# AER-RC/monoRTM

Measured on AMD Instinct MI355X. Metric: (wavenumber x layer x line) optical-depth evals/sec, higher is better.
Workload: dtype f64; 1 GPU; c4: configs[3] whole: 1024 synthetic sonde profiles x 64 layers x 50 channels x 500 lines, f64, profile-sharded over 1 GPU(s): 1024 profiles on this rank; layers=64, wavenumbers=50, lines=500, nmol=7, launch=3 stream launches, parallelism=profile-sharded x1

## Files before the change

monortm_amd/csrc/api.hip:

```cpp
#include <algorithm>
#include <atomic>
#include <chrono>
#include <cmath>
#include <cstdlib>
#include <cstdio>
#include <cstring>
#include <dlfcn.h>
#include <functional>
#include <string>
#include <vector>

#include "device_common.hpp"
#include "line_table.hpp"
#include "modm_plan.hpp"
#include "lineshape.hpp"
#include "tables/monortm_tables.h"

namespace {
using namespace monortm_dev;

thread_local std::string g_init_error;

struct Ctx {
    int device = 0;
    int cus = 256;
    size_t phys_cap = 2ull << 30, far_cap = 1ull << 30;
    std::vector<Ctx *> shards;
    struct Opt : ModmPlanOpt {
        int ms_ablate = 0;
        int ms_prepare = MS_PREPARE_FUSED;
        double jac_dt = MONORTM_JAC_DT, jac_dlnw = MONORTM_JAC_DLNW;
    } opt;
    void *comm = nullptr;
    int comm_rank = 0, comm_world = 1;
    bool has_lines = false;
    int real_kind = 8;
    std::string err;
    monortm::LineTable host;
    DevLines lines{};
    DevTables tables{};
    std::vector<void *> owned;
    int *errflag = nullptr;
    void *partial = nullptr;
    monortm_dev::MwCache mw_cache;
    void *phys = nullptr;
    size_t phys_bytes = 0;
    void *far = nullptr;
    size_t far_bytes = 0;
    double lines_per_cm = 0.;
    bool no_physics_pass = false;
    hipStream_t far_stream = nullptr;
    hipEvent_t far_ev[2] = {nullptr, nullptr};
    double lc_frac = 0.;
    const int *ms_slot_base = nullptr;
    int ms_slot_host[MXMOL + 1] = {0};
    void *ms_scratch = nullptr;
    unsigned short *ms_reach = nullptr;
    size_t ms_scratch_bytes = 0;
    double *osum = nullptr;
    size_t osum_elems = 0;
    DevXsec xs{};
    std::vector<void *> xs_buf;
    struct Stage {
        void *p = nullptr;
        size_t bytes = 0;
    };
    Stage stage[12];
    void *jac_ws = nullptr;
    size_t jac_ws_bytes = 0;
    struct Obs {
        int handle = 0;
        int npath = 0, nwn = 0, nview = 0, nchan = 0;
        void *dev = nullptr;
// ... 74 lines not shown
    bool isint = false, isdbl = false;
    if (!autov) {
        char *end = nullptr;
        iv = strtol(v.c_str(), &end, 10);
        isint = end && end != v.c_str() && *end == '\0';
        end = nullptr;
        dv = strtod(v.c_str(), &end);
        isdbl = end && end != v.c_str() && *end == '\0';
    }
    if (n == "nslice" && (autov || (isint && iv >= 1 && iv <= 16))) c->opt.nslice = autov ? 0 : (int)iv;
    else if (n == "fair" && (autov || (isint && (iv == 0 || iv == 1)))) c->opt.fair = autov ? -1 : (int)iv;
    else if (n == "tile_waves" && (autov || (isint && (iv == 1 || iv == 2 || iv == 4)))) c->opt.tile_waves = autov ? 0 : (int)iv;
    else if (n == "far_levels" && (autov || (isint && iv >= 0 && iv <= FAR_MAXLEV))) c->opt.far_levels = autov ? -1 : (int)iv;
    else if (n == "lines_kernel" && (autov || v == "wn" || v == "ms")) c->opt.lines_ms = autov ? -1 : (v == "ms" ? 1 : 0);
    else if (n == "ms_prepare" && (autov || v == "fused" || v == "passes")) c->opt.ms_prepare = v == "passes" ? MS_PREPARE_PASSES : MS_PREPARE_FUSED;
#ifdef MONORTM_EXPERIMENT
    else if (n == "ms_ablate" && isint && iv >= 0 && iv <= 9) c->opt.ms_ablate = (int)iv;
#endif
    else if (n == "finish" && (autov || v == "generic")) c->opt.finish_generic = autov ? 0 : 1;
    else if (n == "ms_items" && (autov || (isint && (iv == 64 || iv == 128 || iv == 192 || iv == 256)))) c->opt.ms_items = autov ? 0 : (int)iv;
    else if ((n == "jac_dt" || n == "jac_dlnw") && (autov || (isdbl && std::isfinite(dv) && dv > 0. && (n == "jac_dt" || dv < 1.)))) {
        if (n == "jac_dt") c->opt.jac_dt = autov ? MONORTM_JAC_DT : dv;
        else c->opt.jac_dlnw = autov ? MONORTM_JAC_DLNW : dv;
    }
    else { c->err = "unknown option or value: " + n + " = " + v; return MONORTM_EARG; }
    return MONORTM_OK;
}

template <class T>
int upload(Ctx *c, const T *src, size_t n, const T **dst) {
// ... 691 lines not shown
        }
        if (hipGetLastError() != hipSuccess || hipDeviceSynchronize() != hipSuccess) { c->err = "log-ratio tables could not be formed"; return failed(MONORTM_EHIP); }
    }
    void *ef = nullptr;
    if (hipMalloc(&ef, sizeof(int)) != hipSuccess || hipMemset(ef, 0, sizeof(int)) != hipSuccess) { c->err = "hipMalloc(errflag) failed"; return failed(MONORTM_EHIP); }
    c->owned.push_back(ef);
    c->errflag = static_cast<int *>(ef);
    if (hipDeviceSynchronize() != hipSuccess) { c->err = "device set-up failed"; return failed(MONORTM_EHIP); }
    if (hipStreamCreateWithFlags(&c->hs, hipStreamNonBlocking) != hipSuccess ||
        hipHostMalloc(reinterpret_cast<void **>(&c->errflag_host), sizeof(int), hipHostMallocDefault) != hipSuccess) {
        c->err = "stream / pinned flag of the host-buffer entry points could not be created";
        return failed(MONORTM_EHIP);
    }
    if (const char *e = getenv("MONORTM_HOST_TIMING")) c->host_timing = e[0] == '1';
    if (getenv("MONORTM_FINISH_GENERIC")) c->opt.finish_generic = 1;
    for (const char *k : {"lines_kernel", "nslice", "fair", "tile_waves", "far_levels", "ms_items", "ms_prepare",
#ifdef MONORTM_EXPERIMENT
                          "ms_ablate",
#endif
                         }) {
        std::string env = "MONORTM_" + std::string(k);
        for (char &ch : env) ch = (char)toupper((unsigned char)ch);
        if (const char *e = getenv(env.c_str()))
            if (set_option(c, k, e)) { c->err = env + ": " + c->err; return failed(MONORTM_EARG); }
    }
    if (c->host_timing && !g_timing_ctx) {
        g_timing_ctx = c;
        static bool registered = false;
        if (!registered) { atexit([] { if (g_timing_ctx) print_host_timing(g_timing_ctx); }); registered = true; }
    }
    *out = c;
// ... 9 lines not shown
        return;
    }
    print_host_timing(c);
    if (g_timing_ctx == c) g_timing_ctx = nullptr;
    DeviceGuard guard;
    hipSetDevice(c->device);
    for (auto &e : c->events) { hipEventDestroy(e.a); hipEventDestroy(e.b); }
    for (auto &e : c->event_pool) hipEventDestroy(e);
    comm_release(c);
    if (c->hs) hipStreamDestroy(c->hs);
    if (c->errflag_host) hipHostFree(c->errflag_host);
    for (void *p : c->owned) hipFree(p);
    if (c->partial) hipFree(c->partial);
    if (c->osum) hipFree(c->osum);
    if (c->ms_scratch) hipFree(c->ms_scratch);
    for (void *p : c->xs_buf) hipFree(p);
    if (c->phys) hipFree(c->phys);
    if (c->far) hipFree(c->far);
    if (c->far_stream) hipStreamDestroy(c->far_stream);
    for (hipEvent_t e : c->far_ev)
        if (e) hipEventDestroy(e);
    c->mw_cache.release();
    if (c->jac_ws) hipFree(c->jac_ws);
    for (auto &ob : c->obs)
        if (ob.dev) hipFree(ob.dev);
    for (int i = 0; i < 12; i++)
        if (c->stage[i].p) {
            if (i % 2 == 0) hipHostFree(c->stage[i].p);
            else hipFree(c->stage[i].p);
        }
// ... 386 lines not shown
    if (pl.use_ms) {
        HIPCHK(c, grow(&c->ms_scratch, &c->ms_scratch_bytes, lines_ms_scratch(ms, (long long)ms.npg * nlay_max)));
        const size_t nl4 = (std::max<size_t>(c->host.size(), 1) + 3) / 4 * 4;
        if (!c->ms_reach) {
            void *p = nullptr;
            HIPCHK(c, hipMalloc(&p, 6 * nl4));
            c->owned.push_back(p);
            c->ms_reach = static_cast<unsigned short *>(p);
        }
        ms.reach = c->ms_reach;
        ms.near0 = reinterpret_cast<float *>(c->ms_reach + nl4);
        ms.scratch = c->ms_scratch;
        ms.slot_base = c->ms_slot_base;
        ms.ablate = c->opt.ms_ablate;
        ms.prepare = c->opt.ms_prepare;
    }
    const dim3 grid(pl.grid[0], pl.grid[1], pl.grid[2]);
    if (pl.use_ms && pl.ms_nprof < nprof) {
        ModmArgs am = a, aw = a;
        am.nprof = pl.ms_nprof;
        const size_t st = (size_t)pl.ms_nprof * nlay_max;
        auto shift = [](const void *p, size_t elems) { return p ? static_cast<const void *>(static_cast<const double *>(p) + elems) : nullptr; };
        aw.nprof = nprof - pl.ms_nprof;
        aw.P = shift(a.P, st); aw.T = shift(a.T, st); aw.CLW = shift(a.CLW, st); aw.WBRODL = shift(a.WBRODL, st);
        aw.WKL = shift(a.WKL, st * nmol);
        aw.nlay = a.nlay + pl.ms_nprof;
        aw.O = const_cast<void *>(shift(a.O, st * nwn)); aw.O_CLW = const_cast<void *>(shift(a.O_CLW, st * nwn));
        aw.O_BY_MOL = const_cast<void *>(shift(a.O_BY_MOL, st * nmol * nwn));
        aw.OC = const_cast<void *>(shift(a.OC, st * MONORTM_NCONT * nwn));
        aw.osum = a.osum ? a.osum + st * nwn : nullptr;
// ... 888 lines not shown
```

monortm_amd/csrc/device_common.hpp:

```cpp
#pragma once
#include <hip/hip_runtime.h>

#if (defined(FAR_ABL_HOT) || defined(FAR_ABL_STEPS) || defined(FAR_ABL_TRANS) || defined(MONORTM_ABLATE_LOOP) || defined(MONORTM_ABLATE_EVAL) || \
     defined(MONORTM_ABLATE_VOIGT) || defined(MONORTM_ABLATE_ZSEARCH) || defined(MONORTM_ABLATE_EXP4) || defined(MONORTM_ABLATE_COUPLE) ||     \
     defined(MONORTM_NO_CLAMP_GUARD) || defined(MONORTM_NO_UNIFIED) || defined(MONORTM_NO_VSCAN) ||              \
     defined(MONORTM_NO_HALF) || defined(MONORTM_NO_FULL) || defined(MONORTM_NO_CHUNKFAR) || defined(MONORTM_NO_SGL_TSKIP) || defined(LINES_TIMING) || \
     defined(LINES_CLASS_STATS) || defined(MW_TIMING)) &&                                                                                          \
    !defined(MONORTM_EXPERIMENT)
#error "a timing-experiment / A-B switch of monortm_amd is defined: such builds are measurements, not the product - add -DMONORTM_EXPERIMENT=1"
#endif

#include <cstdint>

#include "../../include/monortm_hip.h"

namespace monortm_dev {

#define K_PI 3.1415926535898
#define K_PLANCK 6.62606876E-27
#define K_BOLTZ 1.3806503E-16
#define K_CLIGHT 2.99792458E+10
#define K_AVOGAD 6.02214199E+23
#define K_RADCN1 1.191042722E-12
#define K_RADCN2 1.4387752
// ... 263 lines not shown
constexpr int MS_HOTA_BYTES = 32;
struct MsArgs {
    int G, LPS, CL, nsteps;
    int spp;
    int sa_stride;
    int npg;
    int nslot;
    int inv_cl;
    int inv_lps;
    const int *slot_base;
    void *scratch;
    unsigned short *reach;
    float *near0;
    int ablate;
    int prepare;
};
#define MS_PREPARE_FUSED 0
#define MS_PREPARE_PASSES 1
size_t lines_ms_scratch(const MsArgs &ms, long long nwg);
void launch_lines_ms(const ModmArgs &a, const DevLines &L, const DevTables &tb, const MsArgs &ms, bool ibrd, hipStream_t s);

void launch_physics(const ModmArgs &a, const DevLines &L, const DevTables &tb, int nlines, bool ibrd, hipStream_t s);
void launch_far_plan(const ModmArgs &a, const DevLines &L, const DevTables &tb, hipStream_t s);
void launch_far(const ModmArgs &a, const DevLines &L, const DevTables &tb, double rho_tile, double lines_per_cm, long long *launches,
                hipStream_t s);
void launch_lines(const ModmArgs &a, const DevLines &L, const DevTables &tb, int nw, int wpl, bool ibrd, dim3 grid, size_t dyn_lds,
                  hipStream_t s);
hipError_t launch_finish(const ModmArgs &a, const DevTables &tb, double V1ABS, double V2ABS, int NPTABS, int csize, bool high,
                         bool par, int threads, size_t lds, int lds_sets, hipStream_t s);
void launch_reduce_slices(const ModmArgs &a, hipStream_t s);
void launch_logratio(const double *t296, const double *tlow, double *out, int n, hipStream_t s);
struct MwCache {
    struct Entry {
// ... 28 lines not shown
```

monortm_amd/csrc/lines_ms_kernel.hip:

```cpp
#define MONORTM_EXP_SGPR_CONSTANTS 1
#include "lines_device.hpp"
#include "lines_ms_asm.hpp"
#include "modm_plan.hpp"
#include "ms_reach.hpp"

namespace {
using namespace monortm_dev;

constexpr int WPS = MS_WPS;
#if defined(MONORTM_ABLATE_EXP4) || defined(MONORTM_ABLATE_ZSEARCH) || defined(MONORTM_ABLATE_VOIGT) || defined(MONORTM_NO_CLAMP_GUARD)
constexpr bool MS_HAS_TRIP = false;
#else
constexpr bool MS_HAS_TRIP = true;
#endif
static_assert(MS_REACH_SLOTS == MS_WPS, "ms_reach.hpp forms one bit per wavenumber of a lane");

__device__ __forceinline__ void ms_sync() {
    __builtin_amdgcn_fence(__ATOMIC_RELEASE, "wavefront");
    __builtin_amdgcn_wave_barrier();
    __builtin_amdgcn_fence(__ATOMIC_ACQUIRE, "wavefront");
}
__device__ __forceinline__ void ms_sync_global() {
    __builtin_amdgcn_fence(__ATOMIC_RELEASE, "workgroup");
    __builtin_amdgcn_s_waitcnt(0);
// ... 7 lines not shown
    const ColdLine *gC;
    int item0;
};
struct MsSpec { unsigned long long w[MS_MAXSTEPS]; };
__device__ __forceinline__ bool ms_own(const MsSpec &sp, int item) {
    unsigned long long x = sp.w[0];
#pragma unroll
    for (int t = 1; t < MS_MAXSTEPS; t++) x = ((item >> 6) == t) ? sp.w[t] : x;
    return (x >> (item & 63)) & 1ull;
}
__device__ __forceinline__ HotB ms_hotb(const MsState &st, const MsSpec &sp, int j, const HotA &h) {
    if (ms_own(sp, st.item0 + j)) return st.gB[j];
    return HotB{h.pa, -1., 0., 1.};
}

template <int KIND>
__device__ __forceinline__ void ms_voigt_flush(const HotA *sA, const HotB *gB, const ColdLine *gC, const MsArgs &ms, const unsigned short *vq, int n,
                                               const double (&W)[WPS], int mol, double (&S)[WPS], int *errflag) {
    const int lane = (int)__lane_id();
    const unsigned rec = (lane < n) ? vq[lane] : 0u;
    const int j = (int)((rec >> 9) & 63u), kk = (int)((rec >> 6) & 7u), owner = (int)(rec & 63u);
    double WNi = __shfl(W[0], owner);
#pragma unroll
    for (int k = 1; k < WPS; k++) {
        const double wk = __shfl(W[k], owner);
        WNi = (kk == k) ? wk : WNi;
    }
    double val = 0.;
    if (lane < n) {
        const int so = owner / ms.LPS;
        const HotA h = sA[so * ms.sa_stride + j];
        const HotB b = gB[so * ms.CL + j];
// ... 8 lines not shown
    }
    for (int it = 0; it < n; it++) {
        const int lo = __builtin_amdgcn_readlane(__double2loint(val), it), hi = __builtin_amdgcn_readlane(__double2hiint(val), it);
        const int r = __builtin_amdgcn_readlane((int)rec, it);
        const double v = __hiloint2double(hi, lo);
        if (lane == (r & 63)) {
            const int k = (r >> 6) & 7;
#pragma unroll
            for (int q = 0; q < WPS; q++)
                if (k == q) S[q] += v;
        }
    }
}
template <int KIND>
__device__ __attribute__((noinline)) void ms_voigt_scan(unsigned long long cand, unsigned long long ymask, MsState st, MsSpec sp, const HotA *sA,
                                              const HotB *gB, const ColdLine *gC, MsArgs ms, const double (&W)[WPS], unsigned kvalid, int mol,
                                              double (&S)[WPS], int *errflag, unsigned short *vq) {
    const int lane = (int)__lane_id();
    int nq = 0;
    while (cand) {
        const int j = (int)__builtin_ctzll(cand);
        cand &= cand - 1ull;
        const unsigned ybit = (unsigned)((ymask >> j) & 1ull) << 15;
        const HotA h = st.sA[j];
        const bool own = ms_own(sp, st.item0 + j);
        const double d100 = own ? st.gB[j].d100 : -1.;
        const double cutlim = (KIND == 1) ? h.pa : 25.;
#pragma unroll
        for (int k = 0; k < WPS; k++) {
            const double ad = fabs(W[k] - h.xnu);
            const bool useV = ((kvalid >> k) & 1u) && !(ad > cutlim) && !(ad > d100);
// ... 65 lines not shown
                for (int k = 0; k < WPS; k++) S[k] = uni_single_any<KIND>(cls, h, h.pa, W[k], S[k]);
            }
        }
        j += len;
    }
    const unsigned long long span = ((j1 >= 64) ? ~0ull : ((1ull << j1) - 1ull)) & ~((1ull << j0) - 1ull);
    const unsigned long long cand = V & span;
    bool scan = cand != 0ull;
#ifdef MONORTM_EXPERIMENT
    if (ms.ablate == 4) scan = false;
#endif
    if (scan) {
        double Wt[WPS], St[WPS];
#pragma unroll
        for (int k = 0; k < WPS; k++) { Wt[k] = W[k]; St[k] = S[k]; }
        ms_voigt_scan<KIND>(cand, Y, st, sp, sA, gB, gC, ms, Wt, kvalid, mol, St, errflag, vq);
#pragma unroll
        for (int k = 0; k < WPS; k++) S[k] = St[k];
    }
    {
        int ln = (int)__lane_id();
        asm volatile("" : "+v"(ln));
#pragma unroll
        for (int k = 0; k < WPS; k++) sS[k * 64 + ln] = S[k];
    }
}

__host__ __device__ inline size_t ms_scratch_per_wg(int G, int CL) {
    return ((size_t)G * CL * (sizeof(HotB) + sizeof(ColdLine)) + sizeof(double) * 3 * WPS * 64 + 15) / 16 * 16;
}

// ... 44 lines not shown
struct MsLane { int lane, se, ce, prof, item0; unsigned kvalid; bool act; };
__device__ __forceinline__ MsLane ms_lane(const MsArgs &mc, int pg, const int *sRole) {
    MsLane l;
    l.lane = (int)__lane_id();
    asm volatile("" : "+v"(l.lane));
    const unsigned r = (unsigned)sRole[l.lane];
    l.se = (int)(r & 255u);
    l.ce = (int)((r >> 8) & 255u);
    l.kvalid = (r >> 16) & 255u;
    l.prof = ((r >> 24) & 1u) ? pg * mc.G + l.se : 0;
    l.act = (r >> 25) & 1u;
    l.item0 = (int)(((r >> 26) & 3u) * 64u + ((r >> 28) & 7u) * (unsigned)mc.CL);
    return l;
}

__device__ __attribute__((noinline)) int ms_prologue(const unsigned long long *sKseg, int lay, int pg) {
    extern __shared__ __attribute__((aligned(16))) double dyn_lds[];
    const kseg_t ks = ms_kseg_from(*sKseg);
    const ModmArgs &a = *(const ModmArgs *)ks;
    const DevLines &L = *(const DevLines *)(ks + KA_LINES);
    const DevTables &tb = *(const DevTables *)(ks + KA_TABLES);
    const MsArgs &ms = *(const MsArgs *)(ks + KA_MS);
    const int G = ms.G, LPS = ms.LPS, CL = ms.CL, nmol = a.nmol, nwn = a.nwn, nslot = ms.nslot;
    const MsLds l = ms_lds(dyn_lds, G, ms.sa_stride, nmol, nslot, nullptr);
    const int lane = threadIdx.x;
    const int se_raw = (int)(((unsigned)lane * (unsigned)ms.inv_lps) >> 16);
    const bool lane_in = se_raw < G;
    const int se = lane_in ? se_raw : 0, ce = lane_in ? lane - se_raw * LPS : 0;
    const int prof_e = pg * G + se;
    const bool prof_ok = lane_in && prof_e < a.nprof;
// ... 64 lines not shown
        }
        if (act_e && ce == 0 && !(Tk >= 70. && Tk <= 3000.)) atomicOr(a.errflag, ERRBIT_TEMP);
    }
    if (lane < nmol) { l.sLo[lane] = 0x7fffffff; l.sOff[lane + 1] = 0; }
    for (int i = lane; i < 2 * G; i += 64) l.sA[(i >> 1) * ms.sa_stride + CL + (i & 1)] = HotA{0., 1., 0., 0.};
    ms_sync();

    if (lane == 0) {
        unsigned long long dense = 0ull;
        for (int s = 0; s < G; s++) {
            const double rh = l.sLay[s * 20];
            if (l.sLay[s * 20 + 19] != 0. && !(rh <= MS_REACH_RHO)) dense = 1ull;
        }
        l.sMask[4 + MS_MAXSTEPS + WPS] = dense;
    }
    for (int i = lane; i < G * nmol; i += 64) {
        const int s = i / nmol, m = i - s * nmol, mol = m + 1;
        const double *ly = l.sLay + s * 20;
        if (ly[19] == 0.) continue;
        const double wkq = l.sW[s * nmol + m];
        int lo = L.mol_start[m + 1], hi = L.mol_start[m + 2];
        if (wkq == 0.) continue;
        const double RHORAT = ly[0], WTOT = ly[9], Tk = ly[18];
        if ((mol != 7 || !((L.lc_mask >> 7) & 1ull)) && ((L.sorted_mask >> mol) & 1ull) && WTOT == WTOT && RHORAT == RHORAT && Tk == Tk) {
            const double pad = L.max_abs_shift * fmax(RHORAT, 1.0) + 1e-6;
            const double vlo = l.sWn[0] - 25.0 - pad, vhi = l.sWn[63] + 25.0 + pad;
            int l0 = lo, l1 = hi;
            while (l0 < l1) { const int mid = (l0 + l1) >> 1; if (L.vnu[mid] < vlo) l0 = mid + 1; else l1 = mid; }
            const int first = l0;
            l1 = hi;
// ... 4 lines not shown
        if (hi > lo) {
            atomicMin(&l.sLo[m], lo);
            atomicMax(&l.sOff[m + 1], hi);
        }
    }
    ms_sync();
    if (lane == 0) {
        int acc = 0;
        l.sOff[0] = 0;
        for (int m = 0; m < nmol; m++) {
            const int cnt = (l.sOff[m + 1] > l.sLo[m]) ? l.sOff[m + 1] - l.sLo[m] : 0;
            acc += cnt;
            l.sOff[m + 1] = acc;
        }
    }
    ms_sync();
    for (int i = lane; i < G * nslot; i += 64) {
        const int s = i / nslot, slot = i - s * nslot;
        int m = 0;
        while (m + 1 < nmol && l.sSlot[m + 1] <= slot) m++;
        const int mol = m + 1, iso = slot - l.sSlot[m] + 1;
        const double *ly = l.sLay + s * 20;
        double sc = 0., dop = 0.;
        if (ly[19] != 0. && l.sOff[m + 1] > l.sOff[m]) {
            const double Tk = ly[18];
            if (!(Tk < 70. || Tk > 3000.)) {
                bool bad = false;
                sc = tips_scor(tb.tips_isonm, tb.tips_offset, tb.tips_qoft, tb.tips_q296, mol, iso, Tk, &bad);
                if (bad) atomicOr(a.errflag, ERRBIT_TEMP);
            }
            const double M = tb.smass[(mol - 1) * 9 + iso - 1];
            if (M > 0.) dop = doppler_factor(M, Tk);
        }
        l.sScor[i] = sc;
        l.sDop[i] = dop;
    }
    if (act_e)
        for (int m = 0; m < nmol; m++)
            if (l.sOff[m + 1] == l.sOff[m]) {
#pragma unroll
                for (int k = 0; k < WPS; k++)
                    if ((kvalid >> k) & 1u) obm[(size_t)m * nwn + ce + LPS * k] = 0.;
            }
    ms_sync();
    return l.sOff[nmol];
}

template <int NS>
__device__ __forceinline__ bool ms_prepare_trip(const MsArgs &ms, const MsLds &ld, int nslot, bool lin, int m, int slot0, const LineFields &lf,
                                                float near0) {
#pragma clang fp contract(off)
    const int G = ms.G, CL = ms.CL, spp = ms.spp;
    int lane = (int)__lane_id();
    asm volatile("" : "+v"(lane));
    const int sub = (int)(((unsigned)lane * (unsigned)ms.inv_cl) >> 16), l = lane - sub * CL;
    const bool lane_in = sub < spp;
    const int mol = m + 1, iso = (lf.meta >> 6) & 15;
    const double RADCT = K_PLANCK * K_CLIGHT / K_BOLTZ;
    const double xnu0 = lf.xnu0, s0adj = lf.s0adj, alpf = lf.alfa, delt = lf.pshift, E = lf.epp, XTILD = lf.tmpalf;
    const double RE = RADCT * E;
    double alps = lf.hwhm;
    if (mol == 1 && alps == 0.) alps = 5 * alpf;
    const double near_s = (double)near0 * (1. - 1e-6);
    const int oself = 10 + min(mol, MXBRD) - 1, oslot = slot0 + (iso ? iso - 1 : 0);
    const double w0 = ld.sWn[0], w63 = ld.sWn[63];
    double Xnu[NS], xa[4 * NS], ex[4 * NS];
#pragma unroll
    for (int t = 0; t < NS; t++) {
        const int s = t * spp + sub;
        const double *ly = ld.sLay + ((lane_in & (s < G)) ? s : 0) * 20;
        const double RHORAT = ly[0], lnRT = ly[3], cTk = ly[4], cT0 = ly[5], dTinv = ly[6];
        Xnu[t] = xnu0 + (delt * RHORAT);
        xa[4 * t] = RE * dTinv;
        xa[4 * t + 1] = -(Xnu[t] * cTk);
        xa[4 * t + 2] = -(Xnu[t] * cT0);
        xa[4 * t + 3] = XTILD * lnRT;
    }
    exp_prep_n<4 * NS>(xa, ex);
    bool bad = false;
#pragma unroll
    for (int t = 0; t < NS; t++) {
        const int s = t * spp + sub;
        const bool s_in = lane_in & (s < G);
        const int sc = s_in ? s : 0;
        const double *ly = ld.sLay + sc * 20;
        const bool in = lin & s_in & (ly[19] != 0.);
        const double RHORAT = ly[0], rho_self = ly[oself];
        const double scor = ld.sScor[sc * nslot + oslot], dopfac = ld.sDop[sc * nslot + oslot];
        const double XIPSF = iso ? scor : 0.;
        const double S = s0adj * ex[4 * t] * XIPSF;
        const double STILD = S * ((1 + ex[4 * t + 1]) * frcp_any(Xnu[t] * (1 - ex[4 * t + 2])));
        const double rtx = ex[4 * t + 3];
        const double alfa0i = alpf * rtx, hwhmsi = alps * rtx;
        const double HW = alfa0i * (RHORAT - rho_self) + hwhmsi * rho_self;
        const double HWD = Xnu[t] * dopfac;
        const double c1 = 0., g = 0., wsc = 1.0;
        const double zsum = HW + HWD, zthr = 0.99 * zsum;
        const bool z_gt = HW > zthr * (1. + 1e-12), z_lt = HW < zthr * (1. - 1e-12);
        const double A2 = STILD * HW * (1.0 / K_PI);
        const double HW2 = HW * HW;
        const double p = A2 * frcp_any(625. + HW2);
        const double A2w = A2 * wsc;
        const double pa = (mol == 7) ? 25. : ((mol == 2) ? p : p * ((1. + c1 * 25.) + g)) * wsc;
        const double near_lb = near_s - fabs(Xnu[t] - xnu0) - 1e-9;
        const bool fY = (mol != 7) & (mol != 2) & !((A2w >= 0.) & (HW2 == HW2) & (A2 <= 0.25 * HW2));
        bad |= in & ((!z_gt & !(z_lt & (near_lb > 100. * HWD))) | fY);
        const bool fM2 = (mol != 2) & (w0 + Xnu[t] <= 25.);
        const bool fAL = !(fabs(w0 - Xnu[t]) > 25.) & !(fabs(w63 - Xnu[t]) > 25.);
        if (s_in) {
            ld.sA[s * ms.sa_stride + l] = in ? HotA{Xnu[t], HW2, A2w, pa} : HotA{0., 1., 0., 0.};
            ld.sFlag[s * CL + l] = in ? (unsigned char)((fAL ? 0u : 1u) | (fM2 ? 2u : 0u)) : (unsigned char)0;
        }
    }
    if (__builtin_amdgcn_ballot_w64(bad) != 0ull) return false;
    if ((sub == 0) & (l < NS)) ld.sMask[4 + l] = 0ull;
    return true;
}

template <bool IBRD>
__device__ __forceinline__ void ms_prepare(const unsigned long long *sKseg, int base, int mchunk, int total, HotB *gB, ColdLine *gC) {
    extern __shared__ __attribute__((aligned(16))) double dyn_lds[];
    const kseg_t ks = ms_kseg_from(*sKseg);
    const ModmArgs &a = *(const ModmArgs *)ks;
    const DevLines &L = *(const DevLines *)(ks + KA_LINES);
    const MsArgs &ms = *(const MsArgs *)(ks + KA_MS);
    const int G = ms.G, CL = ms.CL, nmol = a.nmol, nslot = ms.nslot;
    const MsLds ld = ms_lds(dyn_lds, G, ms.sa_stride, nmol, nslot, nullptr);
    const int lane = threadIdx.x;
    const int sub = (int)(((unsigned)lane * (unsigned)ms.inv_cl) >> 16), l = lane - sub * CL;
    const bool lane_in = sub < ms.spp;
    const bool lin = lane_in && base + l < total;
    int m = mchunk, idx = 0, slot0 = 0;
    LineFields lf{0., 0., 0.f, 0.f, 0.f, 0.f, 0.f, 0u};
    float near0 = 0.f;
    if (lin) {
        const int v = base + l;
        while (ld.sOff[m + 1] <= v) m++;
        idx = ld.sLo[m] + (v - ld.sOff[m]);
        slot0 = ld.sSlot[m];
        if constexpr (IBRD) lf.meta = L.meta[idx];
        else lf = load_line_fields(L, idx);
        near0 = ms.near0[idx];
    }
    const uint32_t meta = lf.meta;
    const bool plain = ((meta >> 10) & 3u) == 0u && ((meta >> 13) & 3u) == 0u;
    const bool all_plain = __builtin_amdgcn_ballot_w64(lin && !plain) == 0ull;
    bool done = false;
    if constexpr (MS_HAS_TRIP && !IBRD) {
        if (all_plain && ms.prepare != MS_PREPARE_PASSES && __builtin_amdgcn_ballot_w64(lin && m >= MXBRD) == 0ull) {
            if (ms.nsteps == 3) done = ms_prepare_trip<3>(ms, ld, nslot, lin, m, slot0, lf, near0);
            else if (ms.nsteps == 2) done = ms_prepare_trip<2>(ms, ld, nslot, lin, m, slot0, lf, near0);
        }
    }
#pragma unroll 1
    for (int t = done ? ms.nsteps : 0; t < ms.nsteps; t++) {
        const int s = t * ms.spp + sub;
        const bool s_in = lane_in && s < G;
        const bool in = lin && s_in && ld.sLay[s * 20 + 19] != 0.;
        const int item = s * CL + l;
        HotA hA{0., 1., 0., 0.};
        unsigned flag = 0u;
        bool special = false;
        if (in) {
            int idxp = idx, mp = m;
            uint32_t metap = meta;
            if constexpr (IBRD) asm volatile("" : "+v"(idxp), "+v"(mp), "+v"(metap));
// ... 27 lines not shown
            }
            flag = (fAL ? 0u : 1u) | (fM2 ? 2u : 0u) | (fV ? 4u : 0u) | (fY ? 8u : 0u);
            special = fV || fY;
            if (special) {
                gB[item] = hB;
                gC[item] = cC;
            }
        }
        if (s_in) {
            ld.sA[s * ms.sa_stride + l] = hA;
            ld.sFlag[item] = (unsigned char)flag;
        }
        const unsigned long long bs = __builtin_amdgcn_ballot_w64(special);
        if (lane == 0) ld.sMask[4 + t] = bs;
    }
    ms_sync_global();
    unsigned f = 0u;
    if (lane < CL)
        for (int s = 0; s < G; s++) f |= ld.sFlag[s * CL + lane];
    const unsigned long long NT = __builtin_amdgcn_ballot_w64(f & 1u), M2 = __builtin_amdgcn_ballot_w64(f & 2u),
                             V = __builtin_amdgcn_ballot_w64(f & 4u), Y = __builtin_amdgcn_ballot_w64(f & 8u);
    if (lane == 0) { ld.sMask[0] = NT; ld.sMask[1] = M2; ld.sMask[2] = V; ld.sMask[3] = Y; }
    {
        unsigned r = 0u;
        if (lane < CL && lin) {
            r = ms.reach[idx];
            if ((f & (4u | 8u)) || ld.sMask[4 + MS_MAXSTEPS + WPS] != 0ull) r = 0x1f1fu;
        }
#pragma unroll
        for (int k = 0; k < WPS; k++) {
            const unsigned long long rk = __builtin_amdgcn_ballot_w64((r >> k) & 1u), qk = __builtin_amdgcn_ballot_w64((r >> (8 + k)) & 1u);
            if (lane == 0) { ld.sMask[4 + MS_MAXSTEPS + k] = rk; ld.sMask[4 + MS_MAXSTEPS + WPS + 1 + k] = qk; }
        }
    }
    ms_sync();
}

__global__ void ms_reach_kernel(const double *wn, int nwn, int LPS, DevLines L, int nlines, unsigned short *reach, float *near0) {
    __shared__ double swn[64];
    if (threadIdx.x < 64) swn[threadIdx.x] = wn[min((int)threadIdx.x, max(nwn, 1) - 1)];
    __syncthreads();
    wn = swn;
    nwn = min(nwn, 64);
    const int idx = blockIdx.x * blockDim.x + threadIdx.x;
    if (idx >= nlines) return;
    const uint32_t meta = L.meta[idx];
    const double x = L.vnu[idx], pad = ms_reach_pad(L.max_abs_shift);
    const bool every = ((meta & 63u) == 7u && ((meta >> 10) & 3u)) || !(x == x);
    reach[idx] = (unsigned short)ms_reach_word(wn, nwn, LPS, x, every, pad);
    double best = 0.;
    if (x == x && nwn > 0) {
        int lo = 0, hi = nwn;
        while (lo < hi) {
            const int mid = (lo + hi) >> 1;
            if (wn[mid] < x) lo = mid + 1;
            else hi = mid;
        }
        best = __builtin_inf();
// ... 11 lines not shown
    if (threadIdx.x == 0) sKseg = (unsigned long long)(size_t)__builtin_amdgcn_kernarg_segment_ptr();
    ms_sync();
    const int npg = ms.npg;
    const int lay = a.nlay_max - 1 - (int)blockIdx.x / npg;
    const int pg = (int)blockIdx.x % npg;
    if (blockIdx.x == 0 && threadIdx.x == 0) {
        const kseg_t ks = ms_kseg();
        const ModmArgs &ak = *(const ModmArgs *)ks;
        const DevLines &Lk = *(const DevLines *)(ks + KA_LINES);
        const DevTables &tk = *(const DevTables *)(ks + KA_TABLES);
        const MsArgs &mk = *(const MsArgs *)(ks + KA_MS);
        if (ak.wn != a.wn || ak.errflag != a.errflag || ak.nmol != a.nmol || Lk.vnu != L.vnu || Lk.meta != L.meta || Lk.mol_start[MXMOL + 1] != L.mol_start[MXMOL + 1] ||
            tk.tips_qoft != tb.tips_qoft || tk.smass != tb.smass || mk.scratch != ms.scratch || mk.inv_cl != ms.inv_cl || mk.spp != ms.spp || mk.slot_base != ms.slot_base)
            atomicOr(a.errflag, ERRBIT_ARG);
    }
    const int total = __builtin_amdgcn_readfirstlane(ms_prologue(&sKseg, lay, pg));
    if (total < 0) return;
#ifdef MONORTM_EXPERIMENT
    if (ms.ablate == 1) return;
#endif

    const size_t nitem = (size_t)ms.G * ms.CL;
    HotB *gB = reinterpret_cast<HotB *>(static_cast<char *>(ms.scratch) + (size_t)blockIdx.x * ms_scratch_per_wg(ms.G, ms.CL));
    ColdLine *gC = reinterpret_cast<ColdLine *>(gB + nitem);
    const double *gR = reinterpret_cast<const double *>(gC + nitem);

    bool osum_first = true;
    int mchunk = 0;
    const int CLk = ms.CL;
    const int nchunks = max(1, (total + CLk - 1) / CLk);
    const int fair_t1 = (nchunks + 3) >> 2, fair_t2 = (2 * nchunks + 3) >> 2, fair_t3 = (3 * nchunks + 3) >> 2;
    for (int base = 0, ck = 0; base < total; base += CLk, ck++) {
        if (a.fair) {
            const int q = (ck >= fair_t1) + (ck >= fair_t2) + (ck >= fair_t3);
            if (q <= 0) __builtin_amdgcn_s_setprio(3);
            else if (q == 1) __builtin_amdgcn_s_setprio(2);
            else if (q == 2) __builtin_amdgcn_s_setprio(1);
            else __builtin_amdgcn_s_setprio(0);
        }
        const kseg_t ks = ms_kseg();
        const ModmArgs &ac = *(const ModmArgs *)ks;
        const MsArgs &mc = *(const MsArgs *)(ks + KA_MS);
        const int G = mc.G, LPS = mc.LPS, CL = mc.CL, nmol = ac.nmol, nwn = ac.nwn;
        const MsLds ld = ms_lds(dyn_lds, G, mc.sa_stride, nmol, mc.nslot, const_cast<double *>(gR) + WPS * 64);
        while (mchunk + 1 < nmol && ld.sOff[mchunk + 1] <= base) mchunk++;
        mchunk = __builtin_amdgcn_readfirstlane(mchunk);
        ms_prepare<IBRD>(&sKseg, base, mchunk, total, gB, gC);

#ifdef MONORTM_EXPERIMENT
        if (mc.ablate == 2) continue;
#endif
        MsSpec sp;
#pragma unroll
        for (int t = 0; t < MS_MAXSTEPS; t++) sp.w[t] = uni64(ld.sMask[4 + t]);
        const unsigned long long NT = uni64(ld.sMask[0]), M2 = uni64(ld.sMask[1]), V = uni64(ld.sMask[2]), Y = uni64(ld.sMask[3]);
        unsigned long long RS[WPS], QS[WPS];
#pragma unroll
        for (int k = 0; k < WPS; k++) { RS[k] = uni64(ld.sMask[4 + MS_MAXSTEPS + k]); QS[k] = uni64(ld.sMask[4 + MS_MAXSTEPS + WPS + 1 + k]); }
        for (int m = mchunk; m < nmol; m++) {
            const int o0 = __builtin_amdgcn_readfirstlane(ld.sOff[m]), o1 = __builtin_amdgcn_readfirstlane(ld.sOff[m + 1]);
            if (o1 <= base || o0 >= o1) continue;
            if (o0 >= base + CL) break;
            const int j0 = max(o0, base) - base, j1 = min(o1, base + CL) - base;
            const int mol = m + 1;
            {
                const MsLane ln = ms_lane(mc, pg, ld.sRole);
                const MsState st{ld.sA + ln.se * mc.sa_stride, gB + ln.se * CL, gC + ln.se * CL, ln.item0};
#ifdef MONORTM_EXPERIMENT
                if ((mc.ablate == 3 && (mol == 7 || mol == 2)) || (mc.ablate == 5 && mol != 7 && mol != 2)) continue;
#endif
                if (mol == 7) ms_eval_run<1>(st, sp, ld.sA, gB, gC, mc, NT, M2, V, Y, RS, QS, j0, j1, ld.sWn, ln.ce, ln.kvalid, mol, ld.sS, o0 >= base, ac.errflag, sVq);
                else if (mol == 2) ms_eval_run<2>(st, sp, ld.sA, gB, gC, mc, NT, M2, V, Y, RS, QS, j0, j1, ld.sWn, ln.ce, ln.kvalid, mol, ld.sS, o0 >= base, ac.errflag, sVq);
                else ms_eval_run<0>(st, sp, ld.sA, gB, gC, mc, NT, M2, V, Y, RS, QS, j0, j1, ld.sWn, ln.ce, ln.kvalid, mol, ld.sS, o0 >= base, ac.errflag, sVq);
// ... 29 lines not shown
#pragma unroll
            for (int k = 0; k < WPS; k++)
                if (ce + ms.LPS * k < a.nwn)
                    a.osum[((size_t)prof_e * a.nlay_max + lay) * (size_t)a.nwn + ce + ms.LPS * k] = osum_first ? 0. : os[k * 64 + lane];
        }
    }
}

}

namespace monortm_dev {
static_assert(sizeof(HotA) == MS_HOTA_BYTES, "lines_ms_lds (modm_plan.hpp) sizes the records of a chunk with MS_HOTA_BYTES");
size_t lines_ms_scratch(const MsArgs &ms, long long nwg) { return (size_t)nwg * ms_scratch_per_wg(ms.G, ms.CL); }
void launch_lines_ms(const ModmArgs &a, const DevLines &L, const DevTables &tb, const MsArgs &ms, bool ibrd, hipStream_t s) {
    const int nlines = L.mol_start[MXMOL + 1];
    if (nlines > 0) hipLaunchKernelGGL(ms_reach_kernel, dim3((nlines + 255) / 256), dim3(256), 0, s, a.wn, a.nwn, ms.LPS, L, nlines, ms.reach, ms.near0);
    const dim3 grid((unsigned)(ms.npg * a.nlay_max));
    const size_t lds = lines_ms_lds(ms, a.nmol);
    if (ibrd) hipLaunchKernelGGL((lines_ms_kernel<true>), grid, dim3(64), lds, s, a, L, tb, ms);
    else hipLaunchKernelGGL((lines_ms_kernel<false>), grid, dim3(64), lds, s, a, L, tb, ms);
}
}
```

Measured before the change: 1626 billion evals/s.

## Precompute per-chunk line plan once per launch and skip per-workgroup prepare passes

Extends the reach pre-kernel with extra blocks that compute, once per launch, per-molecule line ranges and per-chunk plain/beyond flags plus reach ballots into a global plan buffer. Workgroups whose layers match the plan assumptions skip the per-layer binary searches and the generic prepare pass. They take the trip fast path and load reach masks from scalar constant memory instead of recomputing them through LDS and a global sync. This trades extra pre-kernel work, a fallback validity check and more branching for less redundant per-workgroup setup.

```diff
diff --git a/monortm_amd/csrc/api.hip b/monortm_amd/csrc/api.hip
--- a/monortm_amd/csrc/api.hip
+++ b/monortm_amd/csrc/api.hip
@@ -29,6 +29,7 @@
     struct Opt : ModmPlanOpt {
         int ms_ablate = 0;
         int ms_prepare = MS_PREPARE_FUSED;
+        int ms_plan = 1;
         double jac_dt = MONORTM_JAC_DT, jac_dlnw = MONORTM_JAC_DLNW;
     } opt;
     void *comm = nullptr;
@@ -57,6 +58,8 @@
     void *ms_scratch = nullptr;
     unsigned short *ms_reach = nullptr;
     size_t ms_scratch_bytes = 0;
+    void *ms_plan = nullptr;
+    size_t ms_plan_words = 0;
     double *osum = nullptr;
     size_t osum_elems = 0;
     DevXsec xs{};
@@ -161,6 +164,7 @@
     else if (n == "far_levels" && (autov || (isint && iv >= 0 && iv <= FAR_MAXLEV))) c->opt.far_levels = autov ? -1 : (int)iv;
     else if (n == "lines_kernel" && (autov || v == "wn" || v == "ms")) c->opt.lines_ms = autov ? -1 : (v == "ms" ? 1 : 0);
     else if (n == "ms_prepare" && (autov || v == "fused" || v == "passes")) c->opt.ms_prepare = v == "passes" ? MS_PREPARE_PASSES : MS_PREPARE_FUSED;
+    else if (n == "ms_plan" && (autov || v == "on" || v == "off")) c->opt.ms_plan = v == "off" ? 0 : 1;
 #ifdef MONORTM_EXPERIMENT
     else if (n == "ms_ablate" && isint && iv >= 0 && iv <= 9) c->opt.ms_ablate = (int)iv;
 #endif
@@ -882,7 +886,7 @@
     }
     if (const char *e = getenv("MONORTM_HOST_TIMING")) c->host_timing = e[0] == '1';
     if (getenv("MONORTM_FINISH_GENERIC")) c->opt.finish_generic = 1;
-    for (const char *k : {"lines_kernel", "nslice", "fair", "tile_waves", "far_levels", "ms_items", "ms_prepare",
+    for (const char *k : {"lines_kernel", "nslice", "fair", "tile_waves", "far_levels", "ms_items", "ms_prepare", "ms_plan",
 #ifdef MONORTM_EXPERIMENT
                           "ms_ablate",
 #endif
@@ -922,6 +926,15 @@
     if (c->partial) hipFree(c->partial);
     if (c->osum) hipFree(c->osum);
     if (c->ms_scratch) hipFree(c->ms_scratch);
+    if (c->ms_plan) {
+#ifdef MONORTM_EXPERIMENT
+        unsigned long long n[4] = {0, 0, 0, 0};
+        if (getenv("MONORTM_MS_PLAN_STATS") && hipDeviceSynchronize() == hipSuccess &&
+            hipMemcpy(n, static_cast<unsigned long long *>(c->ms_plan) + MS_PLAN_CNT, sizeof(n), hipMemcpyDeviceToHost) == hipSuccess)
+            fprintf(stderr, "ms_plan: waves %llu match %llu chunks %llu fast %llu\n", n[0], n[1], n[2], n[3]);
+#endif
+        hipFree(c->ms_plan);
+    }
     for (void *p : c->xs_buf) hipFree(p);
     if (c->phys) hipFree(c->phys);
     if (c->far) hipFree(c->far);
@@ -1338,6 +1351,13 @@
         ms.slot_base = c->ms_slot_base;
         ms.ablate = c->opt.ms_ablate;
         ms.prepare = c->opt.ms_prepare;
+        ms.plan_on = c->opt.ms_plan;
+        if (ms.plan_on) {
+            const size_t had = c->ms_plan_words;
+            HIPCHK(c, grow(&c->ms_plan, &c->ms_plan_words, lines_ms_plan_words((long long)c->host.size(), ms.CL), sizeof(unsigned long long)));
+            if (c->ms_plan_words != had) HIPCHK(c, hipMemsetAsync(c->ms_plan, 0, c->ms_plan_words * sizeof(unsigned long long), s));
+            ms.plan = static_cast<unsigned long long *>(c->ms_plan);
+        }
     }
     const dim3 grid(pl.grid[0], pl.grid[1], pl.grid[2]);
     if (pl.use_ms && pl.ms_nprof < nprof) {
diff --git a/monortm_amd/csrc/device_common.hpp b/monortm_amd/csrc/device_common.hpp
--- a/monortm_amd/csrc/device_common.hpp
+++ b/monortm_amd/csrc/device_common.hpp
@@ -301,9 +301,16 @@
     float *near0;
     int ablate;
     int prepare;
+    int plan_on;
+    unsigned long long *plan;
 };
 #define MS_PREPARE_FUSED 0
 #define MS_PREPARE_PASSES 1
+constexpr int MS_PLAN_OFF = MXMOL;
+constexpr int MS_PLAN_CNT = (2 * MXMOL + 1 + 1) / 2;
+constexpr int MS_PLAN_HEAD = MS_PLAN_CNT + 4;
+constexpr int MS_PLAN_CHUNK = 2 + 2 * MS_WPS;
+inline size_t lines_ms_plan_words(long long nlines, int CL) { return (size_t)MS_PLAN_HEAD + (size_t)MS_PLAN_CHUNK * (size_t)((nlines + CL - 1) / CL); }
 size_t lines_ms_scratch(const MsArgs &ms, long long nwg);
 void launch_lines_ms(const ModmArgs &a, const DevLines &L, const DevTables &tb, const MsArgs &ms, bool ibrd, hipStream_t s);
 
diff --git a/monortm_amd/csrc/lines_ms_kernel.hip b/monortm_amd/csrc/lines_ms_kernel.hip
--- a/monortm_amd/csrc/lines_ms_kernel.hip
+++ b/monortm_amd/csrc/lines_ms_kernel.hip
@@ -45,8 +45,9 @@
     return HotB{h.pa, -1., 0., 1.};
 }
 
+struct MsGeom { int LPS, CL, sa_stride; };
 template <int KIND>
-__device__ __forceinline__ void ms_voigt_flush(const HotA *sA, const HotB *gB, const ColdLine *gC, const MsArgs &ms, const unsigned short *vq, int n,
+__device__ __forceinline__ void ms_voigt_flush(const HotA *sA, const HotB *gB, const ColdLine *gC, const MsGeom &ms, const unsigned short *vq, int n,
                                                const double (&W)[WPS], int mol, double (&S)[WPS], int *errflag) {
     const int lane = (int)__lane_id();
     const unsigned rec = (lane < n) ? vq[lane] : 0u;
@@ -85,7 +86,7 @@
 }
 template <int KIND>
 __device__ __attribute__((noinline)) void ms_voigt_scan(unsigned long long cand, unsigned long long ymask, MsState st, MsSpec sp, const HotA *sA,
-                                              const HotB *gB, const ColdLine *gC, MsArgs ms, const double (&W)[WPS], unsigned kvalid, int mol,
+                                              const HotB *gB, const ColdLine *gC, MsGeom ms, const double (&W)[WPS], unsigned kvalid, int mol,
                                               double (&S)[WPS], int *errflag, unsigned short *vq) {
     const int lane = (int)__lane_id();
     int nq = 0;
@@ -181,7 +182,7 @@
         double Wt[WPS], St[WPS];
 #pragma unroll
         for (int k = 0; k < WPS; k++) { Wt[k] = W[k]; St[k] = S[k]; }
-        ms_voigt_scan<KIND>(cand, Y, st, sp, sA, gB, gC, ms, Wt, kvalid, mol, St, errflag, vq);
+        ms_voigt_scan<KIND>(cand, Y, st, sp, sA, gB, gC, MsGeom{ms.LPS, ms.CL, ms.sa_stride}, Wt, kvalid, mol, St, errflag, vq);
 #pragma unroll
         for (int k = 0; k < WPS; k++) S[k] = St[k];
     }
@@ -256,6 +257,12 @@
     return l;
 }
 
+typedef const __attribute__((address_space(4))) unsigned long long *ms_plan_t;
+__device__ __forceinline__ ms_plan_t ms_plan_chunk(const MsArgs &ms, int ck) {
+    return (ms_plan_t)(size_t)(ms.plan + MS_PLAN_HEAD + (size_t)MS_PLAN_CHUNK * (size_t)ck);
+}
+constexpr int MS_MATCH_BIT = 0x40000000;
+
 __device__ __attribute__((noinline)) int ms_prologue(const unsigned long long *sKseg, int lay, int pg) {
     extern __shared__ __attribute__((aligned(16))) double dyn_lds[];
     const kseg_t ks = ms_kseg_from(*sKseg);
@@ -350,6 +357,33 @@
         }
         l.sMask[4 + MS_MAXSTEPS + WPS] = dense;
     }
+    bool match = false;
+    if (ms.plan_on) {
+        const int *pi = reinterpret_cast<const int *>(ms.plan);
+        bool bad = false;
+        if (lane < G) {
+            const double *ly = l.sLay + lane * 20;
+            bad = ly[19] != 0. && (!(ly[0] <= 1.0) || ly[9] != ly[9] || ly[18] != ly[18]);
+        }
+        if (lane < nmol) {
+            bool has = false;
+            for (int s = 0; s < G; s++) has |= l.sLay[s * 20 + 19] != 0. && l.sW[s * nmol + lane] != 0.;
+            const int o0 = pi[MS_PLAN_OFF + lane], o1 = pi[MS_PLAN_OFF + lane + 1];
+            bad |= !has && o1 > o0;
+            l.sLo[lane] = pi[lane];
+            l.sOff[lane + 1] = o1;
+        }
+        match = __builtin_amdgcn_ballot_w64(bad) == 0ull;
+        if (lane == 0) {
+            l.sOff[0] = 0;
+            if (match) l.sMask[4 + MS_MAXSTEPS + WPS] = 2ull;
+        }
+    }
+    if (!match) {
+    if (ms.plan_on) {
+        if (lane < nmol) { l.sLo[lane] = 0x7fffffff; l.sOff[lane + 1] = 0; }
+        ms_sync();
+    }
     for (int i = lane; i < G * nmol; i += 64) {
         const int s = i / nmol, m = i - s * nmol, mol = m + 1;
         const double *ly = l.sLay + s * 20;
@@ -384,6 +418,7 @@
             l.sOff[m + 1] = acc;
         }
     }
+    }
     ms_sync();
     for (int i = lane; i < G * nslot; i += 64) {
         const int s = i / nslot, slot = i - s * nslot;
@@ -413,12 +448,12 @@
                     if ((kvalid >> k) & 1u) obm[(size_t)m * nwn + ce + LPS * k] = 0.;
             }
     ms_sync();
-    return l.sOff[nmol];
+    return l.sOff[nmol] | ((l.sMask[4 + MS_MAXSTEPS + WPS] & 2ull) ? MS_MATCH_BIT : 0);
 }
 
 template <int NS>
 __device__ __forceinline__ bool ms_prepare_trip(const MsArgs &ms, const MsLds &ld, int nslot, bool lin, int m, int slot0, const LineFields &lf,
-                                                float near0) {
+                                                float near0, bool match) {
 #pragma clang fp contract(off)
     const int G = ms.G, CL = ms.CL, spp = ms.spp;
     int lane = (int)__lane_id();
@@ -448,6 +483,7 @@
     }
     exp_prep_n<4 * NS>(xa, ex);
     bool bad = false;
+    bool anyNT = false, anyM2 = false;
 #pragma unroll
     for (int t = 0; t < NS; t++) {
         const int s = t * spp + sub;
@@ -477,18 +513,28 @@
         bad |= in & ((!z_gt & !(z_lt & (near_lb > 100. * HWD))) | fY);
         const bool fM2 = (mol != 2) & (w0 + Xnu[t] <= 25.);
         const bool fAL = !(fabs(w0 - Xnu[t]) > 25.) & !(fabs(w63 - Xnu[t]) > 25.);
+        anyNT |= in & !fAL;
+        anyM2 |= in & fM2;
         if (s_in) {
             ld.sA[s * ms.sa_stride + l] = in ? HotA{Xnu[t], HW2, A2w, pa} : HotA{0., 1., 0., 0.};
-            ld.sFlag[s * CL + l] = in ? (unsigned char)((fAL ? 0u : 1u) | (fM2 ? 2u : 0u)) : (unsigned char)0;
+            if (!match) ld.sFlag[s * CL + l] = in ? (unsigned char)((fAL ? 0u : 1u) | (fM2 ? 2u : 0u)) : (unsigned char)0;
         }
     }
     if (__builtin_amdgcn_ballot_w64(bad) != 0ull) return false;
+    if (match) {
+        const unsigned long long nt = __builtin_amdgcn_ballot_w64(anyNT), m2 = __builtin_amdgcn_ballot_w64(anyM2);
+        unsigned long long ntf = 0ull, m2f = 0ull;
+        for (int q = 0, sh = 0; q < spp; q++, sh += CL) { ntf |= nt >> sh; m2f |= m2 >> sh; }
+        const unsigned long long low = (CL >= 64) ? ~0ull : ((1ull << CL) - 1ull);
+        if (lane == 0) { ld.sMask[0] = ntf & low; ld.sMask[1] = m2f & low; }
+        return true;
+    }
     if ((sub == 0) & (l < NS)) ld.sMask[4 + l] = 0ull;
     return true;
 }
 
 template <bool IBRD>
-__device__ __forceinline__ void ms_prepare(const unsigned long long *sKseg, int base, int mchunk, int total, HotB *gB, ColdLine *gC) {
+__device__ __forceinline__ bool ms_prepare(const unsigned long long *sKseg, int base, int mchunk, int total, HotB *gB, ColdLine *gC, int ck, bool match) {
     extern __shared__ __attribute__((aligned(16))) double dyn_lds[];
     const kseg_t ks = ms_kseg_from(*sKseg);
     const ModmArgs &a = *(const ModmArgs *)ks;
@@ -514,12 +560,17 @@
     }
     const uint32_t meta = lf.meta;
     const bool plain = ((meta >> 10) & 3u) == 0u && ((meta >> 13) & 3u) == 0u;
-    const bool all_plain = __builtin_amdgcn_ballot_w64(lin && !plain) == 0ull;
+    const unsigned long long pw = match ? ms_plan_chunk(ms, ck)[0] : 0ull;
+    const bool all_plain = match ? (pw & 1ull) != 0ull : __builtin_amdgcn_ballot_w64(lin && !plain) == 0ull;
     bool done = false;
     if constexpr (MS_HAS_TRIP && !IBRD) {
-        if (all_plain && ms.prepare != MS_PREPARE_PASSES && __builtin_amdgcn_ballot_w64(lin && m >= MXBRD) == 0ull) {
-            if (ms.nsteps == 3) done = ms_prepare_trip<3>(ms, ld, nslot, lin, m, slot0, lf, near0);
-            else if (ms.nsteps == 2) done = ms_prepare_trip<2>(ms, ld, nslot, lin, m, slot0, lf, near0);
+        if (all_plain && ms.prepare != MS_PREPARE_PASSES && (match ? (pw & 2ull) == 0ull : __builtin_amdgcn_ballot_w64(lin && m >= MXBRD) == 0ull)) {
+            if (ms.nsteps == 3) done = ms_prepare_trip<3>(ms, ld, nslot, lin, m, slot0, lf, near0, match);
+            else if (ms.nsteps == 2) done = ms_prepare_trip<2>(ms, ld, nslot, lin, m, slot0, lf, near0, match);
+        }
+        if (done && match) {
+            ms_sync();
+            return true;
         }
     }
 #pragma unroll 1
@@ -577,18 +628,21 @@
         const unsigned long long bs = __builtin_amdgcn_ballot_w64(special);
         if (lane == 0) ld.sMask[4 + t] = bs;
     }
+#ifdef MONORTM_EXPERIMENT
+    if (ms.ablate == 6 && done) return false;
+#endif
     ms_sync_global();
     unsigned f = 0u;
     if (lane < CL)
         for (int s = 0; s < G; s++) f |= ld.sFlag[s * CL + lane];
-    const unsigned long long NT = __builtin_amdgcn_ballot_w64(f & 1u), M2 = __builtin_amdgcn_ballot_w64(f & 2u),
+    const unsigned long long cNT = __builtin_amdgcn_ballot_w64(f & 1u), cM2 = __builtin_amdgcn_ballot_w64(f & 2u),
                              V = __builtin_amdgcn_ballot_w64(f & 4u), Y = __builtin_amdgcn_ballot_w64(f & 8u);
-    if (lane == 0) { ld.sMask[0] = NT; ld.sMask[1] = M2; ld.sMask[2] = V; ld.sMask[3] = Y; }
+    if (lane == 0) { ld.sMask[0] = cNT; ld.sMask[1] = cM2; ld.sMask[2] = V; ld.sMask[3] = Y; }
     {
         unsigned r = 0u;
         if (lane < CL && lin) {
             r = ms.reach[idx];
-            if ((f & (4u | 8u)) || ld.sMask[4 + MS_MAXSTEPS + WPS] != 0ull) r = 0x1f1fu;
+            if ((f & (4u | 8u)) || (ld.sMask[4 + MS_MAXSTEPS + WPS] & 1ull) != 0ull) r = 0x1f1fu;
         }
 #pragma unroll
         for (int k = 0; k < WPS; k++) {
@@ -597,14 +651,85 @@
         }
     }
     ms_sync();
-}
-
-__global__ void ms_reach_kernel(const double *wn, int nwn, int LPS, DevLines L, int nlines, unsigned short *reach, float *near0) {
+    return false;
+}
+
+__device__ __forceinline__ void ms_plan_wave(const double *swn, int nwn, int LPS, const DevLines &L, int nmol, int CL, int ck, int nck,
+                                             unsigned long long *plan, int (*pLo)[MXMOL], int (*pOff)[MXMOL + 1]) {
+    const int lane = (int)threadIdx.x & 63, w = (int)threadIdx.x >> 6;
+    int *sLo = pLo[w], *sOff = pOff[w];
+    if (ck >= nck) return;
+    if (lane < nmol) {
+        const int m = lane, mol = m + 1;
+        int lo = L.mol_start[m + 1], hi = L.mol_start[m + 2];
+        if ((mol != 7 || !((L.lc_mask >> 7) & 1ull)) && ((L.sorted_mask >> mol) & 1ull)) {
+            const double pad = L.max_abs_shift * 1.0 + 1e-6;
+            const double vlo = swn[0] - 25.0 - pad, vhi = swn[63] + 25.0 + pad;
+            int l0 = lo, l1 = hi;
+            while (l0 < l1) { const int mid = (l0 + l1) >> 1; if (L.vnu[mid] < vlo) l0 = mid + 1; else l1 = mid; }
+            const int first = l0;
+            l1 = hi;
+            while (l0 < l1) { const int mid = (l0 + l1) >> 1; if (L.vnu[mid] <= vhi) l0 = mid + 1; else l1 = mid; }
+            lo = first;
+            hi = l0;
+        }
+        sLo[m] = (hi > lo) ? lo : 0x7fffffff;
+        sOff[m + 1] = (hi > lo) ? hi - lo : 0;
+    }
+    ms_sync();
+    if (lane == 0) {
+        int acc = 0;
+        sOff[0] = 0;
+        for (int m = 0; m < nmol; m++) { acc += sOff[m + 1]; sOff[m + 1] = acc; }
+    }
+    ms_sync();
+    const int total = sOff[nmol], base = ck * CL;
+    if (ck == 0) {
+        int *pi = reinterpret_cast<int *>(plan);
+        if (lane < nmol) pi[lane] = sLo[lane];
+        if (lane <= nmol) pi[MS_PLAN_OFF + lane] = sOff[lane];
+    }
+    if (base >= total) return;
+    const bool lin = lane < CL && base + lane < total;
+    unsigned r = 0u;
+    bool plain = true, beyond = false;
+    if (lin) {
+        const int v = base + lane;
+        int m = 0;
+        while (sOff[m + 1] <= v) m++;
+        const int idx = sLo[m] + (v - sOff[m]);
+        const uint32_t meta = L.meta[idx];
+        const double x = L.vnu[idx];
+        plain = ((meta >> 10) & 3u) == 0u && ((meta >> 13) & 3u) == 0u;
+        beyond = m >= MXBRD;
+        const bool every = ((meta & 63u) == 7u && ((meta >> 10) & 3u)) || !(x == x);
+        r = ms_reach_word(swn, nwn, LPS, x, every, ms_reach_pad(L.max_abs_shift));
+    }
+    unsigned long long *pc = plan + MS_PLAN_HEAD + (size_t)MS_PLAN_CHUNK * (size_t)ck;
+    const unsigned long long np = __builtin_amdgcn_ballot_w64(lin && !plain), nb = __builtin_amdgcn_ballot_w64(lin && beyond);
+    if (lane == 0) {
+        pc[0] = (np == 0ull ? 1ull : 0ull) | (nb != 0ull ? 2ull : 0ull);
+        pc[1] = 0ull;
+    }
+#pragma unroll
+    for (int k = 0; k < WPS; k++) {
+        const unsigned long long rk = __builtin_amdgcn_ballot_w64((r >> k) & 1u), qk = __builtin_amdgcn_ballot_w64((r >> (8 + k)) & 1u);
+        if (lane == 0) { pc[2 + k] = rk; pc[2 + WPS + k] = qk; }
+    }
+}
+
+__global__ void ms_reach_kernel(const double *wn, int nwn, int LPS, DevLines L, int nlines, unsigned short *reach, float *near0, int reach_blocks,
+                                int nmol, int CL, unsigned long long *plan) {
     __shared__ double swn[64];
+    __shared__ int pLo[4][MXMOL], pOff[4][MXMOL + 1];
     if (threadIdx.x < 64) swn[threadIdx.x] = wn[min((int)threadIdx.x, max(nwn, 1) - 1)];
     __syncthreads();
     wn = swn;
     nwn = min(nwn, 64);
+    if ((int)blockIdx.x >= reach_blocks) {
+        ms_plan_wave(swn, nwn, LPS, L, nmol, CL, ((int)blockIdx.x - reach_blocks) * 4 + ((int)threadIdx.x >> 6), (nlines + CL - 1) / CL, plan, pLo, pOff);
+        return;
+    }
     const int idx = blockIdx.x * blockDim.x + threadIdx.x;
     if (idx >= nlines) return;
     const uint32_t meta = L.meta[idx];
@@ -646,8 +771,14 @@
             tk.tips_qoft != tb.tips_qoft || tk.smass != tb.smass || mk.scratch != ms.scratch || mk.inv_cl != ms.inv_cl || mk.spp != ms.spp || mk.slot_base != ms.slot_base)
             atomicOr(a.errflag, ERRBIT_ARG);
     }
-    const int total = __builtin_amdgcn_readfirstlane(ms_prologue(&sKseg, lay, pg));
-    if (total < 0) return;
+    const int total_m = __builtin_amdgcn_readfirstlane(ms_prologue(&sKseg, lay, pg));
+    if (total_m < 0) return;
+    const int total = total_m & (MS_MATCH_BIT - 1);
+    const bool match = (total_m & MS_MATCH_BIT) != 0;
+#ifdef MONORTM_EXPERIMENT
+    unsigned long long *plan_cnt = ms.plan + MS_PLAN_CNT;
+    if (ms.plan_on && threadIdx.x == 0) { atomicAdd(plan_cnt, 1ull); if (match) atomicAdd(plan_cnt + 1, 1ull); }
+#endif
 #ifdef MONORTM_EXPERIMENT
     if (ms.ablate == 1) return;
 #endif
@@ -677,18 +808,35 @@
         const MsLds ld = ms_lds(dyn_lds, G, mc.sa_stride, nmol, mc.nslot, const_cast<double *>(gR) + WPS * 64);
         while (mchunk + 1 < nmol && ld.sOff[mchunk + 1] <= base) mchunk++;
         mchunk = __builtin_amdgcn_readfirstlane(mchunk);
-        ms_prepare<IBRD>(&sKseg, base, mchunk, total, gB, gC);
+        const bool fast = ms_prepare<IBRD>(&sKseg, base, mchunk, total, gB, gC, ck, match);
 
 #ifdef MONORTM_EXPERIMENT
-        if (mc.ablate == 2) continue;
+        if (mc.ablate == 2 || mc.ablate == 6) continue;
+#endif
+#ifdef MONORTM_EXPERIMENT
+        if (mc.plan_on && threadIdx.x == 0) { atomicAdd(mc.plan + MS_PLAN_CNT + 2, 1ull); if (fast) atomicAdd(mc.plan + MS_PLAN_CNT + 3, 1ull); }
 #endif
         MsSpec sp;
-#pragma unroll
-        for (int t = 0; t < MS_MAXSTEPS; t++) sp.w[t] = uni64(ld.sMask[4 + t]);
-        const unsigned long long NT = uni64(ld.sMask[0]), M2 = uni64(ld.sMask[1]), V = uni64(ld.sMask[2]), Y = uni64(ld.sMask[3]);
-        unsigned long long RS[WPS], QS[WPS];
-#pragma unroll
-        for (int k = 0; k < WPS; k++) { RS[k] = uni64(ld.sMask[4 + MS_MAXSTEPS + k]); QS[k] = uni64(ld.sMask[4 + MS_MAXSTEPS + WPS + 1 + k]); }
+        const unsigned long long NT = uni64(ld.sMask[0]), M2 = uni64(ld.sMask[1]);
+        unsigned long long V = 0ull, Y = 0ull, RS[WPS], QS[WPS];
+        if (fast) {
+            const ms_plan_t pc = ms_plan_chunk(mc, ck);
+#pragma unroll
+            for (int t = 0; t < MS_MAXSTEPS; t++) sp.w[t] = 0ull;
+#pragma unroll
+            for (int k = 0; k < WPS; k++) {
+                ms_plan_t pr = pc + 2 + k, pq = pc + 2 + WPS + k;
+                asm volatile("" : "+s"(pr), "+s"(pq));
+                RS[k] = *pr;
+                QS[k] = *pq;
+            }
+        } else {
+#pragma unroll
+            for (int t = 0; t < MS_MAXSTEPS; t++) sp.w[t] = uni64(ld.sMask[4 + t]);
+            V = uni64(ld.sMask[2]); Y = uni64(ld.sMask[3]);
+#pragma unroll
+            for (int k = 0; k < WPS; k++) { RS[k] = uni64(ld.sMask[4 + MS_MAXSTEPS + k]); QS[k] = uni64(ld.sMask[4 + MS_MAXSTEPS + WPS + 1 + k]); }
+        }
         for (int m = mchunk; m < nmol; m++) {
             const int o0 = __builtin_amdgcn_readfirstlane(ld.sOff[m]), o1 = __builtin_amdgcn_readfirstlane(ld.sOff[m + 1]);
             if (o1 <= base || o0 >= o1) continue;
@@ -748,10 +896,15 @@
 size_t lines_ms_scratch(const MsArgs &ms, long long nwg) { return (size_t)nwg * ms_scratch_per_wg(ms.G, ms.CL); }
 void launch_lines_ms(const ModmArgs &a, const DevLines &L, const DevTables &tb, const MsArgs &ms, bool ibrd, hipStream_t s) {
     const int nlines = L.mol_start[MXMOL + 1];
-    if (nlines > 0) hipLaunchKernelGGL(ms_reach_kernel, dim3((nlines + 255) / 256), dim3(256), 0, s, a.wn, a.nwn, ms.LPS, L, nlines, ms.reach, ms.near0);
+    const int reach_blocks = (nlines + 255) / 256, plan_blocks = (ms.plan_on && ms.plan) ? ((nlines + ms.CL - 1) / ms.CL + 3) / 4 : 0;
+    if (nlines > 0)
+        hipLaunchKernelGGL(ms_reach_kernel, dim3(reach_blocks + plan_blocks), dim3(256), 0, s, a.wn, a.nwn, ms.LPS, L, nlines, ms.reach, ms.near0, reach_blocks,
+                           a.nmol, ms.CL, ms.plan);
     const dim3 grid((unsigned)(ms.npg * a.nlay_max));
     const size_t lds = lines_ms_lds(ms, a.nmol);
-    if (ibrd) hipLaunchKernelGGL((lines_ms_kernel<true>), grid, dim3(64), lds, s, a, L, tb, ms);
-    else hipLaunchKernelGGL((lines_ms_kernel<false>), grid, dim3(64), lds, s, a, L, tb, ms);
-}
-}
+    MsArgs mk = ms;
+    mk.plan_on = (nlines > 0 && plan_blocks > 0) ? 1 : 0;
+    if (ibrd) hipLaunchKernelGGL((lines_ms_kernel<true>), grid, dim3(64), lds, s, a, L, tb, mk);
+    else hipLaunchKernelGGL((lines_ms_kernel<false>), grid, dim3(64), lds, s, a, L, tb, mk);
+}
+}
```

After: 1667 billion evals/s, median of 6. 1.02x the previous value.
